# yangdongchao/RSTnet

Measured on AMD Instinct MI355X. Metric: codec+LM audio frames/sec (24 kHz, 12.5 Hz tokens) at batch=1 and batch=64; RVQ code-index exact-match, higher is better.
Workload: dtype f32 (large GEMMs: operands as three bf16 planes, six bf16 matrix-instruction products per fp32 product, f32 accumulate); 1 GPU; MimiCodec encode->RVQ(8x2048x256)->decode, BASELINE.json configs[1]; batch_per_gpu=64, weights=random-init (rstnet_amd.synth seed 0), parallelism=replica x1, utterances sharded, RCCL weight broadcast only

## Files before the change

rstnet_amd/csrc/b3_common.h:

```cpp
#pragma once
#include "rst_common.h"

typedef short bf16x8 __attribute__((ext_vector_type(8)));
typedef unsigned u32x2 __attribute__((ext_vector_type(2)));
typedef unsigned u32x4 __attribute__((ext_vector_type(4)));
typedef float f32x2 __attribute__((ext_vector_type(2)));
typedef __bf16 bf16x2_t __attribute__((ext_vector_type(2)));

__device__ __forceinline__ unsigned b3_peel(f32x2& v) {
    const unsigned h = __builtin_bit_cast(unsigned, __builtin_convertvector(v, bf16x2_t));
    v[0] -= __uint_as_float(h << 16);
    v[1] -= __uint_as_float(h & 0xffff0000u);
    return h;
}

#define B3_QA {2, 0, 1, 1, 0, 0}
#define B3_QB {0, 2, 1, 0, 1, 0}
```

rstnet_amd/csrc/gemm_win.hip:

```cpp
#include <algorithm>
#include "rst_common.h"
#include "rst_kernels.h"
#include "b3_common.h"

namespace {

constexpr int BK = 32;

template <int TM, int TN, bool FULL = false>
__device__ __forceinline__ void gw_epilogue(const GemmWinParams& p, const f32x16 (&acc)[TM][TN], int m0w, int n0w, int M, int lane) {
    const bool has_res = p.res != nullptr;
#pragma unroll
    for (int j = 0; j < TN; ++j) {
        const int n = n0w + j * 32 + (lane & 31);
        const bool n_ok = FULL || n < p.N;
        const float bias = (p.bias && n_ok) ? p.bias[n] : 0.0f;
        const float scale = (p.scale && n_ok) ? p.scale[n] : 1.0f;
#pragma unroll
        for (int i = 0; i < TM; ++i) {
            const int mb = m0w + i * 32 + 4 * (lane >> 5);
            const long o = (long)mb * p.ldy + n;
            float r[16];
#pragma unroll
            for (int e = 0; e < 16; ++e) {
// ... 488 lines not shown
    constexpr int NT = 128 * NWN;
    constexpr int BM = 128, BN = 64 * NWN;
    constexpr int RA = 512 / NT;
    constexpr int A_PLANE = BM * B3_RS, W_PLANE = DIRW ? 0 : BN * B3_RS;
    constexpr int BUF = 3 * (A_PLANE + W_PLANE);
    constexpr int NSA = B3_SETS_A, NSB = B3_SETS_B;
    static_assert(NSA == 4 && NSB == 2, "the rotation below is written out for four activation sets and two weight sets");
    static_assert(NWN == 2 || NWN == 4, "two or four waves along N");
    extern __shared__ __attribute__((aligned(16))) float smem[];
    short* const lds = reinterpret_cast<short*>(smem);

    const int tid = threadIdx.x;
    const int lane = tid & 63;
    const int wave = tid >> 6;
    const int wm = wave / NWN, wn = wave % NWN;
    const int lrow = b3_row(tid >> 2);
    const int lk = (tid & 3) * 4;
    const int frag_row = lane & 31;
    const int frag_k = (lane >> 5) * 8;

    const int M = p.B * p.T_out;
    const int TC = p.T_in * p.C;
    const int tiles_n = (p.N + BN - 1) / BN;
    const int nk = p.K / B3_KB;

    const int xcd = blockIdx.x & 7;
    const int first = gw_xcd_first(tiles, xcd);
    const int count = gw_xcd_first(tiles, xcd + 1) - first;
    const int stride = ((int)gridDim.x + 7 - xcd) >> 3;
    int l = blockIdx.x >> 3;
    if (l >= count) return;

    struct Ctx {
        unsigned ao[RA];
        int klo[RA], kn[RA];
    };
    auto setup = [&](int m0, Ctx& c) {
#pragma unroll
        for (int j = 0; j < RA; ++j) {
            const int m = m0 + lrow + (NT / 4) * j;
            const int mm = min(m, M - 1);
            const int b = mm / p.T_out;
            const int t = mm - b * p.T_out;
            const int f0 = (t * p.S - p.P) * p.C;
            long off = (long)b * p.x_bstride + f0 + lk;
            if (MASK) {
                int klo = max(0, -f0) / B3_KB, khi = min(p.K, TC - f0) / B3_KB;
                if (m >= M || klo >= khi) {
                    klo = khi = 0;
                    off = lk;
                }
                c.klo[j] = klo;
                c.kn[j] = khi - klo;
                off += (long)klo * B3_KB;
            }
            c.ao[j] = (unsigned)(off * 4);
        }
    };
    auto w_tile = [&](int n0) {
        return DIRW ? (unsigned)(n0 / 32) * (unsigned)nk * 3072u : (unsigned)(n0 / 128) * (unsigned)nk * (unsigned)(B3_WTILE * 2);
    };
    const unsigned wo = DIRW ? (unsigned)(wn * TN) * (unsigned)nk * 3072u + (unsigned)lane * 16u
                             : (unsigned)(((long)(tid >> 8) * nk * B3_WTILE + (tid & 255) * 8) * 2);
    const unsigned wo_blk = (unsigned)nk * 3072u;

    f32x4 ra[NSA][RA];
    int rm[NSA][RA];
    u32x4 rb[NSB][3];
    u32x4 rw[NSB][TN][3];
    const int a_dst = lrow * B3_RS + lk;
    const int b_dst = 3 * A_PLANE + ((tid >> 8) * 128 + b3_row((tid & 255) >> 1)) * B3_RS + (tid & 1) * 8;
    const int a_frag = (wm * TM * 32 + frag_row) * B3_RS + frag_k;
    const int b_frag = 3 * A_PLANE + (wn * TN * 32 + frag_row) * B3_RS + frag_k;

    const __amdgpu_buffer_rsrc_t rs_x = __builtin_amdgcn_make_buffer_rsrc(const_cast<float*>(p.x), 0, 0xffffffff, 0x00020000);
    const __amdgpu_buffer_rsrc_t rs_w = __builtin_amdgcn_make_buffer_rsrc(const_cast<short*>(p.w3), 0, 0xffffffff, 0x00020000);
    auto load_a = [&](auto MM, const Ctx& c, const int kt, f32x4 (&dst)[RA], int (&mask)[RA]) {
        constexpr bool MK = decltype(MM)::value != 0;
#pragma unroll
        for (int j = 0; j < RA; ++j) {
            if (MK) {
                const unsigned d = (unsigned)(kt - c.klo[j]);
                const bool ok = d < (unsigned)c.kn[j];
                mask[j] = ok ? -1 : 0;
                const unsigned vo = c.ao[j] + (ok ? d : 0u) * (B3_KB * 4);
                if (BUFL) dst[j] = __builtin_bit_cast(f32x4, __builtin_amdgcn_raw_buffer_load_b128(rs_x, vo, 0, 0));
                else dst[j] = *reinterpret_cast<const f32x4*>(reinterpret_cast<const char*>(p.x) + vo);
            } else {
                if (BUFL) dst[j] = __builtin_bit_cast(f32x4, __builtin_amdgcn_raw_buffer_load_b128(rs_x, c.ao[j], kt * (B3_KB * 4), 0));
                else dst[j] = *reinterpret_cast<const f32x4*>(reinterpret_cast<const char*>(p.x) + (long)kt * (B3_KB * 4) + c.ao[j]);
            }
        }
    };
    auto load_w = [&](const unsigned wb, const int kt, u32x4 (&dst)[3]) {
#pragma unroll
        for (int q = 0; q < 3; ++q) {
            const unsigned so = wb + (unsigned)kt * (B3_WTILE * 2) + q * (128 * B3_KB * 2);
            if (BUFL) dst[q] = __builtin_amdgcn_raw_buffer_load_b128(rs_w, wo, so, 0);
            else dst[q] = *reinterpret_cast<const u32x4*>(reinterpret_cast<const char*>(p.w3) + so + wo);
        }
    };
    auto load_wq = [&](auto UU, auto QQ, const unsigned wb, const int kt) {
        constexpr int U = decltype(UU)::value, q = decltype(QQ)::value;
#pragma unroll
        for (int j = 0; j < TN; ++j) {
            const unsigned so = wb + (unsigned)kt * 3072u + q * 1024u;
            if (BUFL) rw[U][j][q] = __builtin_amdgcn_raw_buffer_load_b128(rs_w, wo + j * wo_blk, so, 0);
            else rw[U][j][q] = *reinterpret_cast<const u32x4*>(reinterpret_cast<const char*>(p.w3) + so + wo + j * wo_blk);
        }
    };
    auto take_a = [&](auto MM, const f32x4 src, const int mask, f32x2 (&v)[2]) {
        typedef int i32x4 __attribute__((ext_vector_type(4)));
        f32x4 x = src;
        if (decltype(MM)::value != 0) x = __builtin_bit_cast(f32x4, __builtin_bit_cast(i32x4, x) & mask);
        if (ELU) {
            x[0] = rst_elu(x[0]); x[1] = rst_elu(x[1]); x[2] = rst_elu(x[2]); x[3] = rst_elu(x[3]);
        }
        v[0] = f32x2{x[0], x[1]};
        v[1] = f32x2{x[2], x[3]};
    };

    f32x16 acc[TM][TN];
    auto clear = [&]() {
#pragma unroll
        for (int i = 0; i < TM; ++i)
#pragma unroll
            for (int j = 0; j < TN; ++j)
#pragma unroll
                for (int e = 0; e < 16; ++e) acc[i][j][e] = 0.0f;
    };

    auto stage = [&](auto SS, auto MM, const Ctx& c, const int kta, const unsigned bp, const int ktb, const int buf) {
        constexpr int S = decltype(SS)::value;
        constexpr int F = (S + 3) % 4, SB = S % 2, FB = (S + 1) % 2;
        if (DBG != 2 && DBG != 3) {
            if (!DIRW) {
                load_w(bp, ktb, rb[FB]);
                __builtin_amdgcn_sched_barrier(0);
            }
            load_a(MM, c, kta, ra[F], rm[F]);
        }
        bf16x8 fa[TM][3], fb[TN][3];
        const short* rd = lds + buf * BUF;
        short* wr = lds + (buf ^ 1) * BUF;
        constexpr int QA[6] = {2, DIRW ? 1 : 0, DIRW ? 0 : 1, DIRW ? 0 : 1, DIRW ? 1 : 0, 0};
        constexpr int QB[6] = {0, DIRW ? 0 : 2, DIRW ? 0 : 1, DIRW ? 2 : 0, 1, DIRW ? 1 : 0};
        if (DIRW && DBG != 3) {
#pragma unroll
            for (int i = 0; i < TM; ++i) fa[i][2] = *reinterpret_cast<const bf16x8*>(rd + a_frag + 2 * A_PLANE + i * 32 * B3_RS);
#pragma unroll
            for (int i = 0; i < TM; ++i) fa[i][1] = *reinterpret_cast<const bf16x8*>(rd + a_frag + A_PLANE + i * 32 * B3_RS);
#pragma unroll
            for (int i = 0; i < TM; ++i) fa[i][0] = *reinterpret_cast<const bf16x8*>(rd + a_frag + i * 32 * B3_RS);
        } else if (DBG != 3) {
#pragma unroll
            for (int j = 0; j < TN; ++j) fb[j][0] = *reinterpret_cast<const bf16x8*>(rd + b_frag + j * 32 * B3_RS);
#pragma unroll
            for (int i = 0; i < TM; ++i) fa[i][2] = *reinterpret_cast<const bf16x8*>(rd + a_frag + 2 * A_PLANE + i * 32 * B3_RS);
#pragma unroll
            for (int i = 0; i < TM; ++i) fa[i][0] = *reinterpret_cast<const bf16x8*>(rd + a_frag + i * 32 * B3_RS);
#pragma unroll
            for (int j = 0; j < TN; ++j) fb[j][2] = *reinterpret_cast<const bf16x8*>(rd + b_frag + 2 * W_PLANE + j * 32 * B3_RS);
#pragma unroll
            for (int i = 0; i < TM; ++i) fa[i][1] = *reinterpret_cast<const bf16x8*>(rd + a_frag + A_PLANE + i * 32 * B3_RS);
#pragma unroll
            for (int j = 0; j < TN; ++j) fb[j][1] = *reinterpret_cast<const bf16x8*>(rd + b_frag + W_PLANE + j * 32 * B3_RS);
        } else {
#pragma unroll
            for (int q = 0; q < 3; ++q) {
#pragma unroll
                for (int i = 0; i < TM; ++i) fa[i][q] = __builtin_bit_cast(bf16x8, ra[S][0]);
#pragma unroll
                for (int jj = 0; jj < TN; ++jj) fb[jj][q] = __builtin_bit_cast(bf16x8, rb[SB][q]);
            }
        }
        __builtin_amdgcn_sched_barrier(0);

        f32x2 v[RA][2];
        u32x2 h[RA];
        constexpr bool SIDE = DBG != 1 && DBG != 3;
        constexpr int PB = 2 * RA + 1, WOPS = DIRW ? 0 : 3, NOPS = WOPS + 3 * PB;
#pragma unroll
        for (int m = 0; m < 24; ++m) {
            const int t = m >> 2, i = (m >> 1) & 1, j = m & 1;
            if (DIRW && DBG != 3) acc[i][j] = __builtin_amdgcn_mfma_f32_32x32x16_bf16(fa[i][QA[t]], __builtin_bit_cast(bf16x8, rw[SB][j][QB[t]]), acc[i][j], 0, 0, 0);
            else acc[i][j] = __builtin_amdgcn_mfma_f32_32x32x16_bf16(fa[i][QA[t]], fb[j][QB[t]], acc[i][j], 0, 0, 0);
            if (DIRW && DBG != 2 && DBG != 3) {
                if (m == 11) load_wq(b3_int<SB>{}, b3_int<0>{}, bp, ktb);
                if (m == 15) load_wq(b3_int<SB>{}, b3_int<2>{}, bp, ktb);
                if (m == 23) load_wq(b3_int<SB>{}, b3_int<1>{}, bp, ktb);
            }
            if (SIDE && m == 0) {
#pragma unroll
                for (int r = 0; r < RA; ++r) take_a(MM, ra[S][r], rm[S][r], v[r]);
            }
            const int op = RA == 2 ? m - 1 : ((m & 1) ? (m - 1) >> 1 : -1);
            if (SIDE && op >= 0 && op < NOPS) {
                if (op < WOPS) {
                    *reinterpret_cast<u32x4*>(wr + b_dst + op * W_PLANE) = rb[SB][op];
                } else {
                    const int u = op - WOPS;
                    const int q = u / PB, w = u % PB;
                    if (w < 2 * RA) {
                        if (DBG == 5) h[w >> 1][w & 1] = __builtin_bit_cast(unsigned, v[w >> 1][w & 1][0]) + q;
                        else h[w >> 1][w & 1] = b3_peel(v[w >> 1][w & 1]);
                    } else {
#pragma unroll
                        for (int r = 0; r < RA; ++r) *reinterpret_cast<u32x2*>(wr + a_dst + q * A_PLANE + r * (NT / 4) * B3_RS) = h[r];
                    }
                }
            }
            __builtin_amdgcn_sched_barrier(0);
        }
        if (DBG != 4) __syncthreads();
    };

    auto prime = [&](const Ctx& c, const unsigned bp, int buf) {
        short* wr = lds + buf * BUF;
        {
            f32x4 xa[RA];
            int xm[RA];
            u32x4 xb[3];
            load_a(b3_int<MASK>{}, c, 0, xa, xm);
            if (!DIRW) load_w(bp, 0, xb);
#pragma unroll
            for (int j = 0; j < RA; ++j) {
                f32x2 v[2];
                take_a(b3_int<MASK>{}, xa[j], xm[j], v);
#pragma unroll
                for (int q = 0; q < 3; ++q) {
                    u32x2 hh;
                    hh[0] = b3_peel(v[0]);
                    hh[1] = b3_peel(v[1]);
                    *reinterpret_cast<u32x2*>(wr + a_dst + q * A_PLANE + j * (NT / 4) * B3_RS) = hh;
                }
            }
            if (!DIRW) {
#pragma unroll
                for (int q = 0; q < 3; ++q) *reinterpret_cast<u32x4*>(wr + b_dst + q * W_PLANE) = xb[q];
            }
        }
        if (DIRW) {
            load_wq(b3_int<0>{}, b3_int<0>{}, bp, 0); load_wq(b3_int<0>{}, b3_int<2>{}, bp, 0); load_wq(b3_int<0>{}, b3_int<1>{}, bp, 0);
            load_wq(b3_int<1>{}, b3_int<0>{}, bp, 1); load_wq(b3_int<1>{}, b3_int<2>{}, bp, 1); load_wq(b3_int<1>{}, b3_int<1>{}, bp, 1);
        } else {
            load_w(bp, 1, rb[0]);
        }
#pragma unroll
        for (int g = 1; g < 4; ++g) load_a(b3_int<MASK>{}, c, g, ra[g - 1], rm[g - 1]);
        __syncthreads();
    };

    Ctx c;
    int tile = first + l;
    int m0 = (tile / tiles_n) * BM, n0 = (tile % tiles_n) * BN;
    setup(m0, c);
    unsigned bp = w_tile(n0);
    unsigned bpn = bp;
    int kb = 2;
    prime(c, bp, 0);
    for (;;) {
        const int ln = l + stride;
        const bool has_next = ln < count;
        const int tile_n = first + ln;
        const int m0n = (tile_n / tiles_n) * BM, n0n = (tile_n % tiles_n) * BN;
        clear();
        int kf = 4;
        auto cross = [&]() {
            kf = 0;
            if (has_next) {
                setup(m0n, c);
                bpn = w_tile(n0n);
            }
        };
        constexpr b3_int<MASK> MM{};
        for (int kt = 0; kt < nk; kt += 4) {
            if (kf == nk) cross();
            stage(b3_int<0>{}, MM, c, kf, bp, kb, 0);
            stage(b3_int<1>{}, MM, c, kf + 1, bp, kb + 1, 1);
            kb += 2;
            if (kb == nk) {
                kb = 0;
                bp = bpn;
            }
            stage(b3_int<2>{}, MM, c, kf + 2, bp, kb, 0);
            stage(b3_int<3>{}, MM, c, kf + 3, bp, kb + 1, 1);
            kb += 2;
            if (kb == nk) {
                kb = 0;
                bp = bpn;
            }
            kf += 4;
        }
        if (!MASK || (m0 + BM <= M && n0 + BN <= p.N)) gw_epilogue<TM, TN, true>(p, acc, m0 + wm * TM * 32, n0 + wn * TN * 32, M, lane);
        else gw_epilogue<TM, TN, false>(p, acc, m0 + wm * TM * 32, n0 + wn * TN * 32, M, lane);
        if (!has_next) break;
        l = ln;
        tile = tile_n;
        m0 = m0n;
        n0 = n0n;
    }
}

template <bool DIRW>
__global__ __launch_bounds__(256) void gemm_win_b3_pack_kernel(const float* __restrict__ w, short* __restrict__ w3, int N, int K, long total) {
    const long i = (long)blockIdx.x * 256 + threadIdx.x;
    if (i >= total) return;
    const int kq = K / 4;
    const int n = (int)(i / kq);
    const int k = (int)(i % kq) * 4;
    f32x4 v = {0.f, 0.f, 0.f, 0.f};
    if (n < N) v = *reinterpret_cast<const f32x4*>(w + (long)n * K + k);
    f32x2 v0 = {v[0], v[1]}, v1 = {v[2], v[3]};
    short* dst = DIRW ? w3 + ((long)(n / 32) * (K / B3_KB) + k / B3_KB) * (3 * 512) + ((n % 32) + 32 * ((k % B3_KB) / 8)) * 8 + k % 8
                      : w3 + ((long)(n / 128) * (K / B3_KB) + k / B3_KB) * B3_WTILE + b3_slot(n % 128) * B3_KB + k % B3_KB;
#pragma unroll
    for (int q = 0; q < 3; ++q) {
        u32x2 h;
        h[0] = b3_peel(v0);
        h[1] = b3_peel(v1);
        *reinterpret_cast<u32x2*>(dst + q * (DIRW ? 512 : 128 * B3_KB)) = h;
    }
}

static bool b3_dirw() {
    static const int v = rst_knob("RST_B3_DIRW", 1);
    return v != 0;
}

template <int TM, int TN, int WM, int WN, int KB = BK>
int launch_cfg(const GemmWinParams& p, bool vec, hipStream_t stream) {
    constexpr int BM = 32 * TM * WM, BN = 32 * TN * WN;
    const long M = (long)p.B * p.T_out;
    const long tiles = ((M + BM - 1) / BM) * ((p.N + BN - 1) / BN);
    if (tiles <= 0) return RST_OK;
    if (tiles > 0x7fffffffL) {
        rst_set_error("gemm_win: too many tiles (%ld)", tiles);
        return RST_ERR_UNSUPPORTED;
    }
    const size_t lds = 2 * (BM + BN) * (KB + 4) * sizeof(float);
    auto go = [&](auto kern) {
        static RstOncePerDevice attr_once;
        if (attr_once.first()) {
            (void)hipFuncSetAttribute(reinterpret_cast<const void*>(kern), hipFuncAttributeMaxDynamicSharedMemorySize, 128 * 1024);
            (void)hipGetLastError();
        }
        hipLaunchKernelGGL(kern, dim3((unsigned)tiles, (unsigned)(p.split_k > 1 ? p.split_k : 1)), dim3(256), lds, stream, p);
    };
    const bool elu = p.act_in == 1;
    if (vec && elu) go(gemm_win_kernel<TM, TN, WM, WN, true, true, KB>);
    else if (vec) go(gemm_win_kernel<TM, TN, WM, WN, true, false, KB>);
    else if (elu) go(gemm_win_kernel<TM, TN, WM, WN, false, true, KB>);
    else go(gemm_win_kernel<TM, TN, WM, WN, false, false, KB>);
    return rst_check_launch("gemm_win");
}

static int gw_cu_count() {
    return rst_cu_count();
}

template <int KB>
int launch_stream(const GemmWinParams& p, long tiles, hipStream_t stream) {
    if (tiles > 0x7fffffffL) {
        rst_set_error("gemm_win: too many tiles (%ld)", tiles);
        return RST_ERR_UNSUPPORTED;
    }
    const size_t lds = 2 * (128 + 128) * (KB + 4) * sizeof(float);
    static const int per_cu_env = rst_knob("RST_GEMM_STREAM_WGS", 0);
    const int per_cu = per_cu_env > 0 ? per_cu_env : (KB == 16 ? 3 : 2);
    const long resident = (long)per_cu * gw_cu_count();
    const unsigned grid = (unsigned)(tiles < resident ? tiles : resident);
    auto go = [&](auto kern) {
        static RstOncePerDevice attr_once;
        if (attr_once.first()) {
            (void)hipFuncSetAttribute(reinterpret_cast<const void*>(kern), hipFuncAttributeMaxDynamicSharedMemorySize, 128 * 1024);
            (void)hipGetLastError();
        }
        hipLaunchKernelGGL(kern, dim3(grid), dim3(256), lds, stream, p, (int)tiles);
    };
#ifdef RST_ABLATION
    static const int dbg = rst_knob("RST_GEMM_DBG", 0);
    if (KB == 16 && dbg == 1) { go(gemm_win_stream_kernel<false, 16, 1>); return rst_check_launch("gemm_win"); }
    if (KB == 16 && dbg == 5) { go(gemm_win_stream_kernel<false, 16, 5>); return rst_check_launch("gemm_win"); }
#endif
    if (p.act_in == 1) go(gemm_win_stream_kernel<true, KB>);
    else go(gemm_win_stream_kernel<false, KB>);
    return rst_check_launch("gemm_win");
}

template <int NWN>
int launch_stream_b3_cfg(const GemmWinParams& p, hipStream_t stream) {
    constexpr int BN = 64 * NWN;
    const long M = (long)p.B * p.T_out;
    const long tiles = ((M + 127) / 128) * ((p.N + BN - 1) / BN);
    if (tiles > 0x7fffffffL) {
        rst_set_error("gemm_win: too many tiles (%ld)", tiles);
        return RST_ERR_UNSUPPORTED;
    }
    const bool dirw = b3_dirw();
    const size_t lds = 2 * 3 * (128 + (dirw ? 0 : BN)) * B3_RS * sizeof(short);
    static const int per_cu = rst_knob("RST_B3_WGS", NWN == 2 ? 2 : 1);
    const long resident = (long)per_cu * gw_cu_count();
    const unsigned grid = (unsigned)(tiles < resident ? tiles : resident);
    auto go = [&](auto kern) {
        static RstOncePerDevice attr_once;
        if (attr_once.first()) {
            (void)hipFuncSetAttribute(reinterpret_cast<const void*>(kern), hipFuncAttributeMaxDynamicSharedMemorySize, 128 * 1024);
            (void)hipGetLastError();
        }
        hipLaunchKernelGGL(kern, dim3(grid), dim3(128 * NWN), lds, stream, p, (int)tiles);
    };
    bool lean = p.P == 0 && M % 128 == 0 && p.N % BN == 0 && (long)(p.T_out - 1) * p.S * p.C + p.K <= (long)p.T_in * p.C;
#ifdef RST_ABLATION
    static const int force_mask = rst_knob("RST_B3_FORCE_MASK", 0);
    if (force_mask) lean = false;
    static const int dbg = rst_knob("RST_B3_DBG", 0);
    if (dirw && dbg == 1) { go(gemm_win_b3_stream_kernel<false, true, NWN, 1, true, true>); return rst_check_launch("gemm_win_b3"); }
    if (dirw && dbg == 2) { go(gemm_win_b3_stream_kernel<false, true, NWN, 2, true, true>); return rst_check_launch("gemm_win_b3"); }
    if (dirw && dbg == 3) { go(gemm_win_b3_stream_kernel<false, true, NWN, 3, true, true>); return rst_check_launch("gemm_win_b3"); }
    if (dirw && dbg == 4) { go(gemm_win_b3_stream_kernel<false, true, NWN, 4, true, true>); return rst_check_launch("gemm_win_b3"); }
    if (dirw && dbg == 5) { go(gemm_win_b3_stream_kernel<false, true, NWN, 5, true, true>); return rst_check_launch("gemm_win_b3"); }
    static const int bufl = rst_knob("RST_B3_BUF", 1);
    if (!bufl && dirw && p.act_in != 1) {
        if (lean) go(gemm_win_b3_stream_kernel<false, false, NWN, 0, false, true>);
        else go(gemm_win_b3_stream_kernel<false, true, NWN, 0, false, true>);
        return rst_check_launch("gemm_win_b3");
    }
#endif
#ifdef RST_ABLATION
    if (!dirw) {
        if (p.act_in == 1) {
            if (lean) go(gemm_win_b3_stream_kernel<true, false, NWN>);
            else go(gemm_win_b3_stream_kernel<true, true, NWN>);
        } else {
            if (lean) go(gemm_win_b3_stream_kernel<false, false, NWN>);
            else go(gemm_win_b3_stream_kernel<false, true, NWN>);
        }
        return rst_check_launch("gemm_win_b3");
    }
#endif
    if (p.act_in == 1) {
        if (lean) go(gemm_win_b3_stream_kernel<true, false, NWN, 0, true, true>);
        else go(gemm_win_b3_stream_kernel<true, true, NWN, 0, true, true>);
    } else {
        if (lean) go(gemm_win_b3_stream_kernel<false, false, NWN, 0, true, true>);
        else go(gemm_win_b3_stream_kernel<false, true, NWN, 0, true, true>);
    }
    return rst_check_launch("gemm_win_b3");
}

int launch_stream_b3(const GemmWinParams& p, hipStream_t stream) {
    static const int wide_knob = rst_knob("RST_B3_WIDE", 1);
    const int waste = ((p.N + 255) / 256) * 256 - p.N;
    const long wide_tiles = (((long)p.B * p.T_out + 127) / 128) * ((p.N + 255) / 256);
    if (wide_knob && p.N >= 256 && waste * 8 <= p.N && wide_tiles >= 2L * gw_cu_count()) return launch_stream_b3_cfg<4>(p, stream);
    return launch_stream_b3_cfg<2>(p, stream);
}

}

static int gw_tile_cfg(long M, int N) {
    if (N > 64) return M > 4096 ? 0 : 1;
    if (N > 32) return 2;
    return 3;
}
static void gw_tile_dims(int cfg, int& BM, int& BN) {
    BM = cfg == 0 ? 128 : cfg == 1 ? 32 : cfg == 2 ? 128 : 256;
    BN = cfg == 0 ? 128 : cfg == 1 ? 128 : cfg == 2 ? 64 : 32;
}

int rst_gemm_split_plan_impl(long M, int N, int K) {
    if (M <= 0 || M > 4096 || (M <= 32 && N <= 64)) return 1;
    int BM, BN;
    gw_tile_dims(gw_tile_cfg(M, N), BM, BN);
    const long tiles = ((M + BM - 1) / BM) * ((N + BN - 1) / BN);
    const int nk = (K + BK - 1) / BK;
    int s = 1;
    while (tiles * s * 2 <= 256 && nk / (2 * s) >= 2 && s < 64) s *= 2;
    return s;
}

bool rst_gemm_win_b3_shape_ok(int B, int T_in, int T_out, int C, int K, int N, int pad_mode, long x_bstride, bool has_hist) {
    if (B <= 0 || T_in <= 0 || T_out <= 0 || C <= 0 || K <= 0 || N <= 0) return false;
    const long M = (long)B * T_out;
    if (gw_tile_cfg(M, N) != 0) return false;
    if (K % 64 != 0 || C % 16 != 0 || x_bstride % 4 != 0 || has_hist || pad_mode != 0) return false;
    const long x_bytes = ((long)(B - 1) * x_bstride + (long)T_in * C) * 4;
    const long w_bytes = rst_gemm_win_b3_weight_elems_impl(N, K) * 2;
    return x_bytes < 0xfffff000L && w_bytes < 0xfffff000L;
}

int rst_launch_gemm_win(const GemmWinParams& p, hipStream_t stream) {
    RST_REQUIRE(p.B >= 0 && p.T_in >= 0 && p.T_out >= 0 && p.C > 0 && p.K > 0 && p.N > 0 && p.S > 0 && p.P >= 0,
                "gemm_win: bad sizes B=%d T_in=%d T_out=%d C=%d K=%d N=%d S=%d P=%d", p.B, p.T_in, p.T_out, p.C,
                p.K, p.N, p.S, p.P);
    if (p.B == 0 || p.T_out == 0) return RST_OK;
    RST_REQUIRE(p.w && p.y && (p.x || p.T_in == 0), "gemm_win: null pointer");
    RST_REQUIRE((long)p.T_in * p.C < 0x7fffffffL && (long)p.T_out * p.S * p.C < 0x7fffffffL,
                "gemm_win: per-batch activation too large for 32-bit indexing");
    const bool vec = (p.C % 4 == 0) && (p.K % 4 == 0) && (p.x_bstride % 4 == 0) &&
                     ((uintptr_t)p.x % 16 == 0) && ((uintptr_t)p.w % 16 == 0) &&
                     (!p.hist || (uintptr_t)p.hist % 16 == 0);
    const long M = (long)p.B * p.T_out;
    RST_REQUIRE(p.split_k <= 1 || (p.ws && p.counters && M <= 4096), "gemm_win: split-K needs M <= 4096 and the scratch buffers");
    RST_REQUIRE(!p.w3 || gw_tile_cfg(M, p.N) == 0, "gemm_win_b3: %ld x %d is not a large-launch shape (more than 4096 rows, N > 64)", M, p.N);
    switch (gw_tile_cfg(M, p.N)) {
        case 0: {
            const long tiles = ((M + 127) / 128) * ((p.N + 127) / 128);
            static const bool kb32_only = rst_knob("RST_GEMM_KB32", 0) != 0;
            static const bool stream_off = rst_knob("RST_GEMM_STREAM", 1) == 0;
            if (p.w3) {
                RST_REQUIRE(vec && p.split_k <= 1 && (uintptr_t)p.w3 % 16 == 0 &&
                            rst_gemm_win_b3_shape_ok(p.B, p.T_in, p.T_out, p.C, p.K, p.N, p.pad_mode, p.x_bstride, p.hist != nullptr),
                            "gemm_win_b3: shape / alignment not served by the three-plane kernel (B=%d T_in=%d T_out=%d C=%d K=%d N=%d pad=%d "
                            "hist=%d); ask rst_gemm_win_b3_supported", p.B, p.T_in, p.T_out, p.C, p.K, p.N, p.pad_mode, p.hist != nullptr);
                return launch_stream_b3(p, stream);
            }
            static const int under_knob = rst_knob("RST_GEMM_UNDERFILL", 1);
            if (under_knob && tiles < gw_cu_count() && p.split_k <= 1) return launch_cfg<1, 1, 1, 4>(p, vec, stream);
            if (vec && !stream_off && p.split_k <= 1) {
                if (tiles >= 768 && !kb32_only) return launch_stream<16>(p, tiles, stream);
                return launch_stream<32>(p, tiles, stream);
            }
            if (tiles >= 768 && !kb32_only) return launch_cfg<2, 2, 2, 2, 16>(p, vec, stream);
            return launch_cfg<2, 2, 2, 2>(p, vec, stream);
        }
        case 1: return launch_cfg<1, 1, 1, 4>(p, vec, stream);
        case 2: return launch_cfg<1, 2, 4, 1>(p, vec, stream);
        default: return launch_cfg<2, 1, 4, 1>(p, vec, stream);
    }
}

int rst_gemm_split_tiles_impl(long M, int N) {
    int BM, BN;
    gw_tile_dims(gw_tile_cfg(M, N), BM, BN);
    return (int)(((M + BM - 1) / BM) * ((N + BN - 1) / BN));
}

long rst_gemm_win_b3_weight_elems_impl(int N, int K) { return (long)((N + 255) / 256) * 256 * K * 3; }

int rst_launch_gemm_win_b3_pack(const float* w, unsigned short* w3, int N, int K, hipStream_t stream) {
    RST_REQUIRE(w && w3 && N > 0 && K > 0 && K % 16 == 0, "gemm_win_b3_pack_weight: bad arguments (K %% 16 == 0 required, N=%d K=%d)", N, K);
    RST_REQUIRE((uintptr_t)w % 16 == 0 && (uintptr_t)w3 % 16 == 0, "gemm_win_b3_pack_weight: pointers must be 16-byte aligned");
    const long total = (long)((N + 255) / 256) * 256 * (K / 4);
#ifdef RST_ABLATION
    if (!b3_dirw()) {
        hipLaunchKernelGGL(gemm_win_b3_pack_kernel<false>, dim3((unsigned)((total + 255) / 256)), dim3(256), 0, stream, w, reinterpret_cast<short*>(w3), N, K, total);
        return rst_check_launch("gemm_win_b3_pack_weight");
    }
#endif
    hipLaunchKernelGGL(gemm_win_b3_pack_kernel<true>, dim3((unsigned)((total + 255) / 256)), dim3(256), 0, stream, w, reinterpret_cast<short*>(w3), N, K, total);
    return rst_check_launch("gemm_win_b3_pack_weight");
}
```

Baseline: 191,300 frames/s.

## Add tap-sharing b3 GEMM kernel reusing overlapping conv window rows in LDS

Adds a streaming three-plane bf16 GEMM kernel for windowed convolutions with two or three taps where the stride equals the group size. Each tile of output rows loads only 128+R-1 activation rows once into LDS and reuses shifted views for each tap, instead of re-reading and re-splitting the overlapping window for every tap. It is enabled by default through a knob. The cost is more complex tile indexing, slightly fewer useful rows per tile (step 128-(R-1)), an extra LDS halo, and a fixed per-CU residency that skips the existing WGS knob.

Result: faster. 197,000 frames/s (median of 6 runs) (+3.0%).

```diff
diff --git a/rstnet_amd/csrc/b3_common.h b/rstnet_amd/csrc/b3_common.h
--- a/rstnet_amd/csrc/b3_common.h
+++ b/rstnet_amd/csrc/b3_common.h
@@ -14,5 +14,50 @@
     return h;
 }
 
+constexpr int B3_SH_ROWS = 128;
+
+struct B3SharedTile {
+    int b, t0;
+    long m0, mlim;
+};
+struct B3SharedRow {
+    unsigned ao;
+    int klo, kn;
+};
+
+__host__ __device__ __forceinline__ constexpr int b3_shared_step(int R) { return B3_SH_ROWS - (R - 1); }
+__host__ __device__ __forceinline__ constexpr int b3_shared_tiles_per_utt(int T_out, int R) { return (T_out + b3_shared_step(R) - 1) / b3_shared_step(R); }
+
+__host__ __device__ __forceinline__ B3SharedTile b3_shared_tile(int mt, int R, int T_out) {
+    const int tpu = b3_shared_tiles_per_utt(T_out, R), step = b3_shared_step(R);
+    B3SharedTile t;
+    t.b = mt / tpu;
+    t.t0 = (mt - t.b * tpu) * step;
+    t.m0 = (long)t.b * T_out + t.t0;
+    t.mlim = (long)t.b * T_out + (t.t0 + step < T_out ? t.t0 + step : T_out);
+    return t;
+}
+
+__host__ __device__ __forceinline__ B3SharedRow b3_shared_row(const B3SharedTile& t, int r, int R, int G, int TC, long x_bstride, int lk) {
+    const long g = (long)t.t0 + r - (R - 1);
+    const long f0 = g * G;
+    B3SharedRow o;
+    o.klo = 0;
+    if (g < 0 || f0 >= TC) {
+        o.kn = 0;
+        o.ao = (unsigned)(lk * 4);
+    } else {
+        const long left = TC - f0;
+        o.kn = (int)((left < G ? left : (long)G) / 16);
+        o.ao = (unsigned)(((long)t.b * x_bstride + f0 + lk) * 4);
+    }
+    return o;
+}
+
+__host__ __device__ __forceinline__ unsigned b3_shared_load_offset(const B3SharedRow& row, int kt, bool& ok) {
+    ok = (unsigned)kt < (unsigned)row.kn;
+    return row.ao + (ok ? (unsigned)kt : 0u) * 64u;
+}
+
 #define B3_QA {2, 0, 1, 1, 0, 0}
 #define B3_QB {0, 2, 1, 0, 1, 0}
diff --git a/rstnet_amd/csrc/gemm_win.hip b/rstnet_amd/csrc/gemm_win.hip
--- a/rstnet_amd/csrc/gemm_win.hip
+++ b/rstnet_amd/csrc/gemm_win.hip
@@ -814,6 +814,250 @@
     }
 }
 
+template <int TM, int TN>
+__device__ __forceinline__ void gw_epilogue_rows(const GemmWinParams& p, const f32x16 (&acc)[TM][TN], long m0, int rows, int rw, int n0w, int lane) {
+    const bool has_res = p.res != nullptr;
+    const unsigned bytes = (unsigned)rows * (unsigned)p.ldy * 4u;
+    const __amdgpu_buffer_rsrc_t rs_y = __builtin_amdgcn_make_buffer_rsrc(p.y + m0 * p.ldy, 0, bytes, 0x00020000);
+    const __amdgpu_buffer_rsrc_t rs_r = __builtin_amdgcn_make_buffer_rsrc(const_cast<float*>(has_res ? p.res + m0 * p.ldy : p.y), 0, has_res ? bytes : 0u, 0x00020000);
+    const unsigned row_bytes = (unsigned)p.ldy * 4u;
+#pragma unroll
+    for (int j = 0; j < TN; ++j) {
+        const int n = n0w + j * 32 + (lane & 31);
+        const float bias = p.bias ? p.bias[n] : 0.0f;
+        const float scale = p.scale ? p.scale[n] : 1.0f;
+#pragma unroll
+        for (int i = 0; i < TM; ++i) {
+            const unsigned o = (unsigned)(rw + i * 32 + 4 * (lane >> 5)) * row_bytes + (unsigned)n * 4u;
+            float r[16];
+#pragma unroll
+            for (int e = 0; e < 16; ++e) {
+                const unsigned dm = (e & 3) + 8 * (e >> 2);
+                r[e] = has_res ? __uint_as_float(__builtin_amdgcn_raw_buffer_load_b32(rs_r, o + dm * row_bytes, 0, 0)) : 0.0f;
+            }
+#pragma unroll
+            for (int e = 0; e < 16; ++e) {
+                const unsigned dm = (e & 3) + 8 * (e >> 2);
+                float v = acc[i][j][e] + bias;
+                if (p.act_out == 1) v = rst_gelu(v);
+                if (has_res) v = r[e] + scale * v;
+                if (p.act_out == 2) v = rst_elu(v);
+                __builtin_amdgcn_raw_buffer_store_b32(__float_as_uint(v), rs_y, o + dm * row_bytes, 0, 0);
+            }
+        }
+    }
+}
+
+template <bool ELU, int NWN, int R>
+__global__ __launch_bounds__(128 * NWN) __attribute__((amdgpu_waves_per_eu(2, 2))) void gemm_win_b3_stream_shared_kernel(const GemmWinParams p, const int tiles) {
+    constexpr int TM = 2, TN = 2;
+    constexpr int NT = 128 * NWN;
+    constexpr int BN = 64 * NWN;
+    constexpr int RA = 512 / NT;
+    constexpr int A_PLANE = (B3_SH_ROWS + R - 1) * B3_RS;
+    constexpr int BUF = 3 * A_PLANE;
+    constexpr int NSA = B3_SETS_A;
+    static_assert(NSA == 4 && B3_SETS_B == 2, "the rotation below is written out for four activation sets and two weight sets");
+    static_assert(R == 2 || R == 3, "two or three taps");
+    extern __shared__ __attribute__((aligned(16))) float smem[];
+    short* const lds = reinterpret_cast<short*>(smem);
+
+    const int tid = threadIdx.x;
+    const int lane = tid & 63;
+    const int wave = tid >> 6;
+    const int wm = wave / NWN, wn = wave % NWN;
+    const int lrow = b3_row(tid >> 2);
+    const int lk = (tid & 3) * 4;
+    const int frag_row = lane & 31;
+    const int frag_k = (lane >> 5) * 8;
+
+    const int G = p.S * p.C;
+    const int TC = p.T_in * p.C;
+    const int tiles_n = (p.N + BN - 1) / BN;
+    const int nkg = G / B3_KB;
+    const int nk = R * nkg;
+
+    const int xcd = blockIdx.x & 7;
+    const int first = gw_xcd_first(tiles, xcd);
+    const int count = gw_xcd_first(tiles, xcd + 1) - first;
+    const int stride = ((int)gridDim.x + 7 - xcd) >> 3;
+    int l = blockIdx.x >> 3;
+    if (l >= count) return;
+
+    struct Ctx {
+        B3SharedRow row[RA];
+    };
+    auto setup = [&](const int tile, Ctx& c) {
+        const B3SharedTile ti = b3_shared_tile(tile / tiles_n, R, p.T_out);
+#pragma unroll
+        for (int j = 0; j < RA; ++j) c.row[j] = b3_shared_row(ti, lrow + (NT / 4) * j, R, G, TC, p.x_bstride, lk);
+    };
+    auto w_tile = [&](int n0) { return (unsigned)(n0 / 32) * (unsigned)nk * 3072u; };
+    const unsigned wo = (unsigned)(wn * TN) * (unsigned)nk * 3072u + (unsigned)lane * 16u;
+    const unsigned wo_blk = (unsigned)nk * 3072u;
+
+    f32x4 ra[NSA][RA];
+    int rm[NSA][RA];
+    u32x4 rw[2][TN][3];
+    const int a_dst = lrow * B3_RS + lk;
+    const int a_frag = (wm * TM * 32 + frag_row) * B3_RS + frag_k;
+
+    const __amdgpu_buffer_rsrc_t rs_x = __builtin_amdgcn_make_buffer_rsrc(const_cast<float*>(p.x), 0, 0xffffffff, 0x00020000);
+    const __amdgpu_buffer_rsrc_t rs_w = __builtin_amdgcn_make_buffer_rsrc(const_cast<short*>(p.w3), 0, 0xffffffff, 0x00020000);
+    auto load_a = [&](const Ctx& c, const int kt, f32x4 (&dst)[RA], int (&mask)[RA]) {
+#pragma unroll
+        for (int j = 0; j < RA; ++j) {
+            bool ok;
+            const unsigned vo = b3_shared_load_offset(c.row[j], kt, ok);
+            mask[j] = ok ? -1 : 0;
+            dst[j] = __builtin_bit_cast(f32x4, __builtin_amdgcn_raw_buffer_load_b128(rs_x, vo, 0, 0));
+        }
+    };
+    auto load_wq = [&](const int u, const int q, const unsigned wb, const int pk) {
+#pragma unroll
+        for (int j = 0; j < TN; ++j) {
+            const unsigned so = wb + (unsigned)pk * 3072u + q * 1024u;
+            rw[u][j][q] = __builtin_amdgcn_raw_buffer_load_b128(rs_w, wo + j * wo_blk, so, 0);
+        }
+    };
+    auto take_a = [&](const f32x4 src, const int mask, f32x2 (&v)[2]) {
+        typedef int i32x4 __attribute__((ext_vector_type(4)));
+        f32x4 x = __builtin_bit_cast(f32x4, __builtin_bit_cast(i32x4, src) & mask);
+        if (ELU) {
+            x[0] = rst_elu(x[0]); x[1] = rst_elu(x[1]); x[2] = rst_elu(x[2]); x[3] = rst_elu(x[3]);
+        }
+        v[0] = f32x2{x[0], x[1]};
+        v[1] = f32x2{x[2], x[3]};
+    };
+
+    f32x16 acc[TM][TN];
+    auto clear = [&]() {
+#pragma unroll
+        for (int i = 0; i < TM; ++i)
+#pragma unroll
+            for (int j = 0; j < TN; ++j)
+#pragma unroll
+                for (int e = 0; e < 16; ++e) acc[i][j][e] = 0.0f;
+    };
+
+    auto stage = [&](auto SS, const Ctx& c, const int kta, const unsigned bp, const unsigned bpn, const int kt, const int buf) {
+        constexpr int S = decltype(SS)::value;
+        constexpr int F = (S + 3) % 4;
+        load_a(c, kta, ra[F], rm[F]);
+        bf16x8 fa[TM][3];
+        const short* rd = lds + buf * BUF + a_frag;
+        short* wr = lds + (buf ^ 1) * BUF + a_dst;
+        constexpr int QA[6] = {2, 1, 0, 0, 1, 0};
+        constexpr int QB[6] = {0, 0, 0, 2, 1, 1};
+#pragma unroll
+        for (int q = 2; q >= 0; --q)
+#pragma unroll
+            for (int i = 0; i < TM; ++i) fa[i][q] = *reinterpret_cast<const bf16x8*>(rd + q * A_PLANE + i * 32 * B3_RS);
+        __builtin_amdgcn_sched_barrier(0);
+
+        f32x2 v[RA][2];
+        u32x2 hh[RA];
+        constexpr int PB = 2 * RA + 1, NOPS = 3 * PB, SP = R * (RA == 2 ? 1 : 2);
+#pragma unroll
+        for (int mm = 0; mm < 24 * R; ++mm) {
+            const int h = mm / 24, m = mm % 24;
+            const int t = m >> 2, i = (m >> 1) & 1, j = m & 1;
+            const int u = (R * S + h) & 1;
+            acc[i][j] = __builtin_amdgcn_mfma_f32_32x32x16_bf16(fa[i][QA[t]], __builtin_bit_cast(bf16x8, rw[u][j][QB[t]]), acc[i][j], 0, 0, 0);
+            if (m == 11 || m == 15 || m == 23) {
+                const int h2 = (h + 2) % R, dk = (h + 2) / R;
+                const bool over = dk != 0 && kt + dk == nkg;
+                load_wq(u, m == 11 ? 0 : (m == 15 ? 2 : 1), over ? bpn : bp, (over ? 0 : kt + dk) + h2 * nkg);
+            }
+            if (h + 1 < R && (m == 3 || m == 19 || m == 23)) {
+                const int q = m == 3 ? 2 : (m == 19 ? 1 : 0);
+#pragma unroll
+                for (int ii = 0; ii < TM; ++ii) fa[ii][q] = *reinterpret_cast<const bf16x8*>(rd + (h + 1) * B3_RS + q * A_PLANE + ii * 32 * B3_RS);
+            }
+            if (mm == 0) {
+#pragma unroll
+                for (int r = 0; r < RA; ++r) take_a(ra[S][r], rm[S][r], v[r]);
+            }
+            const int op = (mm >= 1 && (mm - 1) % SP == 0) ? (mm - 1) / SP : -1;
+            if (op >= 0 && op < NOPS) {
+                const int q = op / PB, w = op % PB;
+                if (w < 2 * RA) {
+                    hh[w >> 1][w & 1] = b3_peel(v[w >> 1][w & 1]);
+                } else {
+#pragma unroll
+                    for (int r = 0; r < RA; ++r) *reinterpret_cast<u32x2*>(wr + q * A_PLANE + r * (NT / 4) * B3_RS) = hh[r];
+                }
+            }
+            __builtin_amdgcn_sched_barrier(0);
+        }
+        __syncthreads();
+    };
+
+    if (tid < 2 * 3 * (R - 1) * 3) {
+        const int piece = tid % 3, row = tid / 3;
+        const int b = row / (3 * (R - 1)), q = (row / (R - 1)) % 3, e = row % (R - 1);
+        *reinterpret_cast<u32x4*>(lds + b * BUF + q * A_PLANE + (B3_SH_ROWS + e) * B3_RS + piece * 8) = u32x4{0u, 0u, 0u, 0u};
+    }
+
+    Ctx c;
+    int tile = first + l;
+    int n0 = (tile % tiles_n) * BN;
+    setup(tile, c);
+    unsigned bp = w_tile(n0);
+    unsigned bpn = bp;
+    {
+        f32x4 xa[RA];
+        int xm[RA];
+        load_a(c, 0, xa, xm);
+#pragma unroll
+        for (int j = 0; j < RA; ++j) {
+            f32x2 v[2];
+            take_a(xa[j], xm[j], v);
+#pragma unroll
+            for (int q = 0; q < 3; ++q) {
+                u32x2 hh;
+                hh[0] = b3_peel(v[0]);
+                hh[1] = b3_peel(v[1]);
+                *reinterpret_cast<u32x2*>(lds + a_dst + q * A_PLANE + j * (NT / 4) * B3_RS) = hh;
+            }
+        }
+        load_wq(0, 0, bp, 0); load_wq(0, 2, bp, 0); load_wq(0, 1, bp, 0);
+        load_wq(1, 0, bp, nkg); load_wq(1, 2, bp, nkg); load_wq(1, 1, bp, nkg);
+#pragma unroll
+        for (int g = 1; g < 4; ++g) load_a(c, g, ra[g - 1], rm[g - 1]);
+        __syncthreads();
+    }
+    for (;;) {
+        const int ln = l + stride;
+        const bool has_next = ln < count;
+        const int tile_n = first + ln;
+        const B3SharedTile ti = b3_shared_tile(tile / tiles_n, R, p.T_out);
+        clear();
+        int kf = 4;
+        for (int kt = 0; kt < nkg; kt += 4) {
+            if (kf == nkg) {
+                kf = 0;
+                if (has_next) {
+                    setup(tile_n, c);
+                    bpn = w_tile((tile_n % tiles_n) * BN);
+                }
+            }
+            stage(b3_int<0>{}, c, kf, bp, bpn, kt, 0);
+            stage(b3_int<1>{}, c, kf + 1, bp, bpn, kt + 1, 1);
+            stage(b3_int<2>{}, c, kf + 2, bp, bpn, kt + 2, 0);
+            stage(b3_int<3>{}, c, kf + 3, bp, bpn, kt + 3, 1);
+            kf += 4;
+        }
+        bp = bpn;
+        if (n0 + BN <= p.N) gw_epilogue_rows<TM, TN>(p, acc, ti.m0, (int)(ti.mlim - ti.m0), wm * TM * 32, n0 + wn * TN * 32, lane);
+        else gw_epilogue<TM, TN, false>(p, acc, (int)ti.m0 + wm * TM * 32, n0 + wn * TN * 32, (int)ti.mlim, lane);
+        if (!has_next) break;
+        l = ln;
+        tile = tile_n;
+        n0 = (tile % tiles_n) * BN;
+    }
+}
+
 template <bool DIRW>
 __global__ __launch_bounds__(256) void gemm_win_b3_pack_kernel(const float* __restrict__ w, short* __restrict__ w3, int N, int K, long total) {
     const long i = (long)blockIdx.x * 256 + threadIdx.x;
@@ -898,6 +1142,30 @@
     if (p.act_in == 1) go(gemm_win_stream_kernel<true, KB>);
     else go(gemm_win_stream_kernel<false, KB>);
     return rst_check_launch("gemm_win");
+}
+
+static int b3_shared_taps(const GemmWinParams& p) {
+    const long G = (long)p.S * p.C;
+    if (G % 64 != 0 || p.K % G != 0) return 0;
+    const long R = p.K / G;
+    if ((R != 2 && R != 3) || p.P != (R - 1) * p.S) return 0;
+    return (int)R;
+}
+
+template <int NWN, int R>
+int launch_shared_b3_cfg(const GemmWinParams& p, hipStream_t stream) {
+    constexpr int BN = 64 * NWN;
+    const long tiles = (long)p.B * b3_shared_tiles_per_utt(p.T_out, R) * ((p.N + BN - 1) / BN);
+    if (tiles > 0x7fffffffL) {
+        rst_set_error("gemm_win: too many tiles (%ld)", tiles);
+        return RST_ERR_UNSUPPORTED;
+    }
+    const size_t lds = 2 * 3 * (B3_SH_ROWS + R - 1) * B3_RS * sizeof(short);
+    const long resident = (long)(NWN == 2 ? 2 : 1) * gw_cu_count();
+    const unsigned grid = (unsigned)(tiles < resident ? tiles : resident);
+    if (p.act_in == 1) hipLaunchKernelGGL((gemm_win_b3_stream_shared_kernel<true, NWN, R>), dim3(grid), dim3(128 * NWN), lds, stream, p, (int)tiles);
+    else hipLaunchKernelGGL((gemm_win_b3_stream_shared_kernel<false, NWN, R>), dim3(grid), dim3(128 * NWN), lds, stream, p, (int)tiles);
+    return rst_check_launch("gemm_win_b3");
 }
 
 template <int NWN>
@@ -951,6 +1219,12 @@
         return rst_check_launch("gemm_win_b3");
     }
 #endif
+    static const int share = rst_knob("RST_B3_SHARE", 1);
+    if (share) {
+        const int taps = b3_shared_taps(p);
+        if (taps == 2) return launch_shared_b3_cfg<NWN, 2>(p, stream);
+        if (taps == 3) return launch_shared_b3_cfg<NWN, 3>(p, stream);
+    }
     if (p.act_in == 1) {
         if (lean) go(gemm_win_b3_stream_kernel<true, false, NWN, 0, true, true>);
         else go(gemm_win_b3_stream_kernel<true, true, NWN, 0, true, true>);
```
